# bytedance/ps-lite

Measured on AMD Instinct MI355X. Metric: push+pull GB/s per worker + p50 round-trip µs, 1 MB & 64 MB, at 1/2/4/8 GPUs, higher is better.
Workload: dtype fp32; 1 GPU; model=dense push+pull (ps-lite test_benchmark PUSH_PULL), global_batch=128, seq_len=67108864, parallelism=byteps-joint x1 (worker+server per GPU), mode=dense, msg_bytes=67108864, batch_keys=False, overlap=True, op=assign

## Files before the change

### csrc/gpu_plane.cc

```cpp
#include "gpu_plane.h"

#include <fcntl.h>
#include <hip/hip_runtime.h>
#include <semaphore.h>
#include <sys/prctl.h>
#include <time.h>
#include <unistd.h>

#include <cstring>

#include "hip_pool.h"
#include "host_par.h"
#include "host_pool.h"
#include "kernels.h"
#include "postoffice.h"
#include "wire.h"

namespace xps {

static const size_t kInlineMax = 4096;

#define XPS_HIP_CHECK(cmd)                                                            \
  do {                                                                                \
    hipError_t e_ = (cmd);                                                            \
    XPS_CHECK(e_ == hipSuccess) << "HIP error: " << hipGetErrorString(e_) << " in " #cmd; \
  } while (0)

std::atomic<uint64_t> g_zero_copy_recv{0};
std::atomic<uint64_t> g_fused_assign{0};

bool FusedAssignEnabled() {
  static const bool on = Environment::Get()->GetInt("XPS_FUSED_ASSIGN", 1) != 0;
  return on;
}

namespace {
std::mutex g_map_mu;
struct HandleKey {
  char h[kIpcHandleBytes];
  bool operator==(const HandleKey& o) const { return memcmp(h, o.h, kIpcHandleBytes) == 0; }
};
struct HandleHash {
  size_t operator()(const HandleKey& k) const {
    size_t v = 1469598103934665603ull;
    for (char c : k.h) {
      v ^= static_cast<unsigned char>(c);
      v *= 1099511628211ull;
    }
    return v;
  }
};
std::unordered_map<HandleKey, void*, HandleHash> g_mapped;

class IpcOpenLock {
 public:
  IpcOpenLock() {
    sem_ = sem_open("/xps_ipc_open_lock", O_CREAT, 0600, 1);
  }
  void Lock() {
// ... 4 lines not shown
    if (sem_timedwait(sem_, &ts) != 0) {
      XPS_LOG(Warning) << "ipc-open lock timeout; proceeding unlocked";
      timed_out_ = true;
    }
  }
  void Unlock() {
    if (sem_ != SEM_FAILED && !timed_out_) sem_post(sem_);
    timed_out_ = false;
  }

 private:
  sem_t* sem_ = SEM_FAILED;
  bool timed_out_ = false;
};
IpcOpenLock g_ipc_lock;
}

GpuPlane::GpuPlane(Postoffice* po, int device) : po_(po), device_(device) {
  my_host_hash_ = HostHash();
  inline_deliver_ = Environment::Get()->GetInt("XPS_INLINE_HANDLER", 1) != 0;
  lanes_ = Environment::Get()->GetInt("XPS_STREAMS_PER_PEER", 2);
  if (lanes_ < 1) lanes_ = 1;
  if (lanes_ > 2) lanes_ = 2;
}

GpuPlane::~GpuPlane() { Stop(); }

void GpuPlane::FillSelf(Node* self) {
  static std::once_flag gc_once;
  std::call_once(gc_once, [] { HostShmPool::GcStaleSegments(); });
  self->dev_id = device_;
  auto* pool = HbmPool::Get();
  if (device_ >= 0 && pool->initialized()) {
    self->pool_capacity = pool->capacity();
    self->pool_slab_bytes = pool->slab_bytes();
    self->pool_handles.resize(pool->slab_count());
    for (size_t i = 0; i < pool->slab_count(); ++i) {
      memcpy(self->pool_handles[i].data(), pool->slab_handle(i), kIpcHandleBytes);
    }
  }
  auto* hpool = HostShmPool::Get();
  hpool->Init(self->shm_uid);
  self->host_pool_uid = hpool->uid();
  self->host_pool_capacity = hpool->capacity();
  if (!started_) {
    auto* env = Environment::Get();
// ... 1 lines not shown
      XPS_CHECK(in_ring_.Create(self->shm_uid)) << "cannot create shm ring";
    }
    started_ = true;
    if (!env->GetInt("XPS_PROBE_NO_POLL", 0)) {
      poll_running_ = true;
      poll_thread_ = std::thread([this] { RingPollLoop(); });
    }
    if (device_ >= 0 && !env->GetInt("XPS_PROBE_NO_COMP", 0)) {
      comp_thread_ = std::thread([this] { CompletionLoop(); });
    }
  }
}

void GpuPlane::Stop() {
  if (stop_.exchange(true)) return;
  PrintStageStats(device_ >= 0 ? "gpu plane" : "host plane");
  if (poll_thread_.joinable()) poll_thread_.join();
  if (comp_thread_.joinable()) comp_thread_.join();
  {
    std::lock_guard<std::mutex> lk(local_mu_);
    for (auto& lm : local_q_) po_->van()->Deliver(std::move(lm.first));
    local_q_.clear();
  }
  {
    std::lock_guard<std::mutex> lk(pend_mu_);
    for (auto& kv : pending_) {
      for (auto& p : kv.second) {
        (void)hipEventSynchronize(p.ev);
        if (p.local_po) {
          DeliverLocal(p.local_po, p.resend, p.bytes);
          (void)hipEventDestroy(p.ev);
          continue;
        }
        Peer* peer = GetPeer(p.peer_id);
        auto ring = peer ? RingOf(peer) : nullptr;
        bool sent = ring && ring->Push(p.payload.data(),
                                       static_cast<uint32_t>(p.payload.size()));
        if (!sent) {
          (void)po_->van()->SendOverTcp(p.resend, p.peer_id);
        }
        (void)hipEventDestroy(p.ev);
      }
    }
    pending_.clear();
  }
  in_ring_.CloseAndUnlink();
  HostShmPool::Get()->Unlink();
  std::lock_guard<std::mutex> lk(ev_mu_);
  for (auto ev : event_pool_) (void)hipEventDestroy(ev);
  event_pool_.clear();
// ... 158 lines not shown
  std::lock_guard<std::mutex> lk(p->mu);
  p->slab_bases = std::move(bases);
  return !p->slab_bases.empty();
}

char* GpuPlane::ResolvePeer(Peer* p, uint64_t global_off, uint64_t len) {
  if (!ImportPeerSlabs(p)) return nullptr;
  uint64_t slab_bytes = p->node.pool_slab_bytes;
  if (slab_bytes == 0) return nullptr;
  size_t idx = static_cast<size_t>(global_off / slab_bytes);
  uint64_t local = global_off % slab_bytes;
  std::lock_guard<std::mutex> lk(p->mu);
  if (idx >= p->slab_bases.size() || len > slab_bytes - local) {
    XPS_LOG(Warning) << "peer offset out of bounds: off=" << global_off << " len=" << len
                     << " slab=" << idx;
    return nullptr;
  }
  return static_cast<char*>(p->slab_bases[idx]) + local;
}

hipStream_t GpuPlane::StreamLane(int node_id, int lane) {
  if (lane >= lanes_) lane = lanes_ - 1;
  Peer* p = GetPeer(node_id);
  hipStream_t s = p->streams[lane].load(std::memory_order_acquire);
  if (s) return s;
  std::lock_guard<std::mutex> lk(p->mu);
  s = p->streams[lane].load(std::memory_order_relaxed);
  if (!s) {
    XPS_HIP_CHECK(hipSetDevice(device_));
    XPS_HIP_CHECK(hipStreamCreateWithFlags(&s, hipStreamNonBlocking));
    p->streams[lane].store(s, std::memory_order_release);
  }
  return s;
}

hipStream_t GpuPlane::StreamForPeer(int node_id) { return StreamLane(node_id, 0); }

hipStream_t GpuPlane::PullStreamForPeer(int node_id) {
  Peer* p = GetPeer(node_id);
  if (lanes_ < 2 || p->node.dev_id == device_) return StreamLane(node_id, 0);
  return StreamLane(node_id, 1);
}

std::vector<std::tuple<int, int64_t, int64_t>> GpuPlane::PeerBytes() {
  std::vector<std::tuple<int, int64_t, int64_t>> out;
  std::shared_lock<std::shared_timed_mutex> lk(peers_mu_);
  for (auto& kv : peers_) {
    int64_t tx = kv.second->tx_bytes.load(std::memory_order_relaxed);
    int64_t rx = kv.second->rx_bytes.load(std::memory_order_relaxed);
    if (tx || rx) out.emplace_back(kv.first, tx, rx);
  }
  return out;
}

hipEvent_t GpuPlane::GetEvent() {
  {
    std::lock_guard<std::mutex> lk(ev_mu_);
    if (!event_pool_.empty()) {
      hipEvent_t ev = event_pool_.back();
      event_pool_.pop_back();
      return ev;
    }
  }
// ... 153 lines not shown
  }
  pending_count_.fetch_add(1);
  p->rx_bytes.fetch_add(bytes, std::memory_order_relaxed);
  return true;
}

bool GpuPlane::EntryPushPull(Message& msg, Peer* p, int64_t* bytes_out) {
  if (!FusedAssignEnabled()) return false;
  if (!(msg.meta.option & kOptPullAddr) || (msg.meta.option & kOptHostAddr)) return false;
  static const bool local_one_sided =
      Environment::Get()->GetInt("XPS_LOCAL_ONE_SIDED", 0) != 0;
  Postoffice* elpo = LocalPeer(p);
  GpuPlane* rplane =
      elpo ? dynamic_cast<GpuPlane*>(elpo->van() ? elpo->van()->plane() : nullptr) : nullptr;
  bool can = elpo ? (local_one_sided && rplane != nullptr) : EnsureRing(p);
  if (!can) return false;
  SArray<char> vals = msg.data[1];
  size_t len = vals.size();
  if (len == 0) return false;
  char* entry = ResolvePeer(p, msg.meta.entry_addr, len);
  char* dst = static_cast<char*>(HbmPool::Get()->PtrOf(msg.meta.addr, len));
  if (!entry || !dst || !kern::Disjoint3(entry, dst, vals.data(), len)) return false;
  XPS_STAGE(entry_push_pull);
  hipStream_t stream = elpo ? rplane->StreamForPeer(po_->node_id()) : StreamForPeer(p->node.id);
  XPS_HIP_CHECK(hipSetDevice(device_));
  kern::DenseAssign2(entry, dst, vals.data(), len, stream);
  g_fused_assign.fetch_add(1, std::memory_order_relaxed);
  g_zero_copy_recv.fetch_add(1, std::memory_order_relaxed);
  Message meta_msg;
  meta_msg.meta = msg.meta;
  meta_msg.meta.option |= kOptInPlace;
  meta_msg.meta.val_len = static_cast<int64_t>(len);
  meta_msg.meta.data_type.clear();
  for (size_t i = 0; i < msg.data.size(); ++i) {
    if (i == 1 || msg.data[i].on_device()) continue;
    meta_msg.data.push_back(msg.data[i]);
    meta_msg.meta.data_type.push_back(msg.meta.data_type[i]);
  }
  int64_t bytes = 64 + static_cast<int64_t>(len);
  Message keepalive;
  keepalive.data.push_back(vals);
  std::string payload;
  if (!elpo) {
    std::vector<char> br(meta_msg.data.size(), 0);
    XPS_CHECK(Serialize(meta_msg, br, &payload));
  }
  hipEvent_t ev = GetEvent();
  XPS_HIP_CHECK(hipEventRecord(ev, stream));
  {
    std::lock_guard<std::mutex> lk(pend_mu_);
    pending_[p->node.id].push_back(Pending{ev, p->node.id, std::move(payload),
                                           std::move(meta_msg), std::move(keepalive), bytes,
                                           elpo});
  }
  pending_count_.fetch_add(1);
  p->tx_bytes.fetch_add(bytes, std::memory_order_relaxed);
  *bytes_out = bytes;
  return true;
}

void GpuPlane::EnqueueLocal(Message msg, int64_t bytes) {
  {
    std::lock_guard<std::mutex> lk(local_mu_);
    local_q_.emplace_back(std::move(msg), bytes);
  }
  local_count_.fetch_add(1, std::memory_order_release);
}

int64_t GpuPlane::SendLocal(Message& msg, Peer* p, Postoffice* lpo) {
  XPS_STAGE(plane_send_local);
  bool response = !msg.meta.request;
  int64_t bytes = 64;
  for (auto& d : msg.data) bytes += static_cast<int64_t>(d.size());

  if (response && msg.meta.pull && msg.data.size() > 1 && !msg.data[1].on_device() &&
      msg.data[1].size() > 0 && (msg.meta.option & kOptPullAddr) &&
// ... 44 lines not shown
      if (i == 1 || msg.data[i].on_device()) continue;
      meta_msg.data.push_back(msg.data[i]);
      meta_msg.meta.data_type.push_back(msg.meta.data_type[i]);
    }
    msg.data.clear();
    Message keepalive;
    keepalive.data.push_back(vals);
    hipEvent_t ev = GetEvent();
    XPS_HIP_CHECK(hipEventRecord(ev, stream));
    {
      std::lock_guard<std::mutex> lk(pend_mu_);
      pending_[p->node.id].push_back(Pending{ev, p->node.id, std::string(),
                                             std::move(meta_msg), std::move(keepalive), bytes,
                                             lpo});
    }
    pending_count_.fetch_add(1);
    p->tx_bytes.fetch_add(bytes, std::memory_order_relaxed);
    return bytes;
  }

  bool kernel_less_ack = KernelLessAck(msg);
  if (response && device_ >= 0 && !kernel_less_ack) {
    XPS_STAGE(local_defer);
    hipStream_t stream = (msg.meta.option & kOptPullLane) ? PullStreamForPeer(p->node.id)
                                                          : StreamForPeer(p->node.id);
    hipEvent_t ev = GetEvent();
    XPS_HIP_CHECK(hipSetDevice(device_));
    XPS_HIP_CHECK(hipEventRecord(ev, stream));
    Message resend = msg;
    {
      std::lock_guard<std::mutex> lk(pend_mu_);
      pending_[p->node.id].push_back(Pending{ev, p->node.id, std::string(), std::move(resend),
                                             Message(), bytes, lpo});
    }
    pending_count_.fetch_add(1);
  } else {
    Message copy = msg;
    if (response) {
      for (auto& d : copy.data) {
        if (!d.on_device() && d.size()) {
          SArray<char> snap(d.size());
          memcpy(snap.data(), d.data(), d.size());
          d = snap;
        }
      }
    }
    DeliverLocal(lpo, copy, bytes);
  }
  p->tx_bytes.fetch_add(bytes, std::memory_order_relaxed);
  return bytes;
}

int64_t GpuPlane::Send(Message& msg, const Node& peer_node) {
  XPS_STAGE(plane_send);
  XPS_VLOG(3) << "plane send -> " << peer_node.id << ": " << msg.DebugString();
  Peer* p = GetPeer(peer_node.id);
// ... 195 lines not shown
  pending_count_.fetch_add(1);
  XPS_VLOG(3) << "deferred send queued -> " << peer_id;
}

void GpuPlane::CompletionLoop() {
  XPS_HIP_CHECK(hipSetDevice(device_));
  prctl(PR_SET_TIMERSLACK, 1000);
  const int kSpin = Environment::Get()->GetInt("XPS_POLL_SPIN", 200000);
  int idle = 0;
  std::vector<int> ids;
  while (!stop_.load()) {
    bool did = false;
    if (pending_count_.load(std::memory_order_acquire) > 0) {
      ids.clear();
      {
        std::lock_guard<std::mutex> lk(pend_mu_);
        for (auto& kv : pending_) {
          if (!kv.second.empty()) ids.push_back(kv.first);
        }
      }
      for (int id : ids) {
        while (!stop_.load()) {
          hipEvent_t front_ev = nullptr;
          {
            std::lock_guard<std::mutex> lk(pend_mu_);
            auto& dq = pending_[id];
            if (dq.empty()) break;
            front_ev = dq.front().ev;
          }
          hipError_t e = hipEventQuery(front_ev);
          if (e == hipErrorNotReady) break;
          XPS_STAGE(defer_release);
          XPS_CHECK(e == hipSuccess) << "hipEventQuery: " << hipGetErrorString(e);
          Pending front;
          {
            std::lock_guard<std::mutex> lk(pend_mu_);
            auto& dq = pending_[id];
            front = std::move(dq.front());
            dq.pop_front();
          }
          pending_count_.fetch_sub(1);
          if (front.local_po) {
            DeliverLocal(front.local_po, front.resend, front.bytes);
            PutEvent(front.ev);
            did = true;
            continue;
          }
          Peer* peer = GetPeer(front.peer_id);
          auto ring = peer ? RingOf(peer) : nullptr;
          bool sent = ring && ring->Push(front.payload.data(),
                                         static_cast<uint32_t>(front.payload.size()));
          if (sent) {
            XPS_VLOG(3) << "deferred send done -> " << front.peer_id;
          } else {
            XPS_LOG(Warning) << "deferred plane send failed -> " << front.peer_id
                             << "; falling back to TCP";
            if (po_->van()->SendOverTcp(front.resend, front.peer_id) < 0) {
              XPS_LOG(Warning) << "TCP fallback to " << front.peer_id
                               << " failed too (peer dead?)";
            }
          }
          PutEvent(front.ev);
          did = true;
        }
      }
    }
    if (did) {
      idle = 0;
    } else if (++idle > kSpin) {
      usleep(20);
    }
  }
}

void GpuPlane::RingPollLoop() {
  if (device_ >= 0) XPS_HIP_CHECK(hipSetDevice(device_));
  prctl(PR_SET_TIMERSLACK, 1000);
  const int kSpin = Environment::Get()->GetInt("XPS_POLL_SPIN", 200000);
  std::vector<char> buf(ShmRing::MaxPayload());
  int idle = 0;
  std::deque<std::pair<Message, int64_t>> local;
  while (!stop_.load()) {
    if (local_count_.load(std::memory_order_acquire) > 0) {
      {
        std::lock_guard<std::mutex> lk(local_mu_);
// ... 98 lines not shown
```

### csrc/gpu_plane.h

```cpp
#pragma once

#include <hip/hip_runtime.h>

#include <atomic>
#include <deque>
#include <memory>
#include <shared_mutex>
#include <thread>
#include <tuple>
#include <unordered_map>
#include <vector>

#include "shm_ring.h"
#include "van.h"

namespace xps {

extern std::atomic<uint64_t> g_zero_copy_recv;
extern std::atomic<uint64_t> g_fused_assign;
bool FusedAssignEnabled();

class Postoffice;

class GpuPlane : public DataPlane {
 public:
  GpuPlane(Postoffice* po, int device);
  ~GpuPlane() override;

  void FillSelf(Node* self) override;
  void ImportPeers() override;
  bool CanSend(const Message& msg, const Node& peer) override;
  int64_t Send(Message& msg, const Node& peer) override;
  void OnPeer(const Node& peer) override;
  void Stop() override;

  hipStream_t StreamForPeer(int node_id);
  hipStream_t PullStreamForPeer(int node_id);
  int lanes() const { return lanes_; }
  std::vector<std::tuple<int, int64_t, int64_t>> PeerBytes();
  int device() const { return device_; }

  bool LocalPullRead(int peer_id, void* dst, uint64_t entry_off, size_t len, Message resp);
  hipEvent_t GetEvent();
  void PutEvent(hipEvent_t ev);
  char* PeerDst(int peer_id, uint64_t global_off, uint64_t len) {
    return ResolvePeer(GetPeer(peer_id), global_off, len);
  }

 private:
  struct Peer {
    Node node;
    std::atomic<Postoffice*> local_po{nullptr};
    std::shared_ptr<ShmRing> ring;
    bool ring_tried = false;
    std::atomic<bool> ring_ok{false};
    std::vector<void*> slab_bases;
    bool pool_tried = false;
    std::atomic<hipStream_t> streams[2] = {{nullptr}, {nullptr}};
    std::atomic<int64_t> tx_bytes{0};
    std::atomic<int64_t> rx_bytes{0};
    std::mutex mu;
  };

  struct Pending {
    hipEvent_t ev;
    int peer_id;
    std::string payload;
    Message resend;
    Message keepalive;
    int64_t bytes;
    Postoffice* local_po = nullptr;
  };

  Peer* GetPeer(int id);
  Postoffice* LocalPeer(Peer* p);
  int64_t SendLocal(Message& msg, Peer* p, Postoffice* lpo);
  void DeliverLocal(Postoffice* lpo, Message& msg, int64_t bytes);
  void EnqueueLocal(Message msg, int64_t bytes);
  bool EnsureRing(Peer* p);
  std::shared_ptr<ShmRing> RingOf(Peer* p);
  bool ImportPeerSlabs(Peer* p);
  char* ResolvePeer(Peer* p, uint64_t global_off, uint64_t len);
  bool Serialize(const Message& msg, const std::vector<char>& by_ref, std::string* out);
  void RingPollLoop();
  void CompletionLoop();
  hipStream_t StreamLane(int node_id, int lane);
  bool EntryPushPull(Message& msg, Peer* p, int64_t* bytes_out);
  void DeferSendInternal(Peer* p, int peer_id, hipStream_t stream, Message resend,
                         Message keepalive, std::string payload, int64_t bytes);

  Postoffice* po_;
  int device_;
  int lanes_ = 2;
  uint64_t my_host_hash_;
  ShmRing in_ring_;
  bool started_ = false;
  bool inline_deliver_ = true;

  std::shared_timed_mutex peers_mu_;
  std::unordered_map<int, std::unique_ptr<Peer>> peers_;

  std::thread poll_thread_;
  std::thread comp_thread_;
  std::atomic<bool> stop_{false};

  std::mutex pend_mu_;
  std::unordered_map<int, std::deque<Pending>> pending_;
  std::atomic<int> pending_count_{0};

  std::mutex local_mu_;
  std::deque<std::pair<Message, int64_t>> local_q_;
  std::atomic<int> local_count_{0};
  bool poll_running_ = false;

  std::mutex ev_mu_;
  std::vector<hipEvent_t> event_pool_;
// ... 6 lines not shown
```

### csrc/kernels.h

```cpp
#pragma once

#include <cstddef>
#include <cstdint>

#include <hip/hip_runtime.h>

namespace xps {
namespace kern {

void DenseAssign(void* dst, const void* src, size_t nbytes, hipStream_t s);
void DenseAssign2(void* dst0, void* dst1, const void* src, size_t nbytes, hipStream_t s,
                  int grid_cap = 0);
inline bool Disjoint3(const void* a, const void* b, const void* c, size_t len) {
  auto apart = [len](const void* x, const void* y) {
    uintptr_t p = reinterpret_cast<uintptr_t>(x), q = reinterpret_cast<uintptr_t>(y);
    return p + len <= q || q + len <= p;
  };
  return apart(a, b) && apart(a, c) && apart(b, c);
}
void DenseSumF32(float* dst, const float* src, size_t n, hipStream_t s);
void DenseSumBf16(uint16_t* dst, const uint16_t* src, size_t n, hipStream_t s);
void BatchedSumBf16(const struct CopyDesc* descs_host, int n, hipStream_t s);
void SparseGatherF32(const float* table, const uint64_t* rows_dev, size_t nrows, size_t row_len,
                     float* out, hipStream_t s, int key_shift = 0, uint64_t row_base = 0,
                     uint64_t table_rows = ~0ull);
void SparseScatterAddF32(float* table, const uint64_t* rows_dev, size_t nrows, size_t row_len,
                         const float* src, bool atomic, hipStream_t s, int key_shift = 0,
                         uint64_t row_base = 0, uint64_t table_rows = ~0ull);
void SparseScatterAssignF32(float* table, const uint64_t* rows_dev, size_t nrows, size_t row_len,
                            const float* src, hipStream_t s, int key_shift = 0,
                            uint64_t row_base = 0, uint64_t table_rows = ~0ull);

static const int kMaxBatch = 64;
struct CopyDesc {
  void* dst;
  const void* src;
  size_t nbytes;
};
void BatchedAssign(const CopyDesc* descs_host, int n, hipStream_t s);
void BatchedSumF32(const CopyDesc* descs_host, int n, hipStream_t s);

}
}
```

### csrc/kernels.hip

```cpp
#include <hip/hip_runtime.h>

#include <algorithm>
#include <cstdlib>

#include "kernels.h"

namespace xps {
namespace kern {

namespace {

constexpr int kBlock = 256;

inline int GridFor(size_t work_items, int cap = 8192) {
  size_t g = (work_items + kBlock - 1) / kBlock;
  if (g > static_cast<size_t>(cap)) g = cap;
  if (g == 0) g = 1;
  return static_cast<int>(g);
}

__global__ void assign_kernel(uint4* __restrict__ dst, const uint4* __restrict__ src, size_t n4) {
  size_t i = blockIdx.x * static_cast<size_t>(blockDim.x) + threadIdx.x;
  size_t stride = static_cast<size_t>(gridDim.x) * blockDim.x;
  for (; i < n4; i += stride) dst[i] = src[i];
// ... 229 lines not shown
      float4 b = *src;
      a.x += b.x;
      a.y += b.y;
      a.z += b.z;
      a.w += b.w;
      *dst = a;
    } else if (kOp == 2) {
      uint4* dst = reinterpret_cast<uint4*>(da.d[seg].dst) + local;
      const uint4* src = reinterpret_cast<const uint4*>(da.d[seg].src) + local;
      uint4 a = *dst;
      uint4 b = *src;
      a.x = bf16x2_sum(a.x, b.x);
      a.y = bf16x2_sum(a.y, b.y);
      a.z = bf16x2_sum(a.z, b.z);
      a.w = bf16x2_sum(a.w, b.w);
      *dst = a;
    } else {
      reinterpret_cast<uint4*>(da.d[seg].dst)[local] =
          reinterpret_cast<const uint4*>(da.d[seg].src)[local];
    }
  }
}

__global__ void batched_assign_kernel(DescArray da) {
  for (int seg = 0; seg < da.n; ++seg) {
    uint4* dst = reinterpret_cast<uint4*>(da.d[seg].dst);
    const uint4* src = reinterpret_cast<const uint4*>(da.d[seg].src);
    size_t n4 = da.d[seg].nbytes / 16;
    size_t i = blockIdx.x * static_cast<size_t>(blockDim.x) + threadIdx.x;
    size_t stride = static_cast<size_t>(gridDim.x) * blockDim.x;
    for (; i < n4; i += stride) dst[i] = src[i];
  }
}

__global__ void batched_sum_kernel_bf16(DescArray da) {
  for (int seg = 0; seg < da.n; ++seg) {
    uint4* dst = reinterpret_cast<uint4*>(da.d[seg].dst);
    const uint4* src = reinterpret_cast<const uint4*>(da.d[seg].src);
    size_t n8 = da.d[seg].nbytes / 16;
    size_t i = blockIdx.x * static_cast<size_t>(blockDim.x) + threadIdx.x;
    size_t stride = static_cast<size_t>(gridDim.x) * blockDim.x;
    for (; i < n8; i += stride) {
      uint4 d = dst[i];
      uint4 s = src[i];
      d.x = bf16x2_sum(d.x, s.x);
      d.y = bf16x2_sum(d.y, s.y);
// ... 53 lines not shown
    int grid = static_cast<int>((acc + cpb - 1) / cpb);
    hipLaunchKernelGGL((batched_balanced_kernel<kOp>), dim3(grid), dim3(kBlock), 0, s, da,
                       cpb);
  }
}

}

void BatchedAssign(const CopyDesc* descs_host, int n, hipStream_t s) {
  if (BalancedBatchEnabled()) {
    LaunchBalanced<0>(descs_host, n, s);
    return;
  }
  size_t total = 0;
  for (int i = 0; i < n; ++i) total += descs_host[i].nbytes;
  DescArray da{};
  for (int off = 0; off < n; off += kMaxBatch) {
    da.n = std::min(n - off, kMaxBatch);
    for (int i = 0; i < da.n; ++i) da.d[i] = descs_host[off + i];
    hipLaunchKernelGGL(batched_assign_kernel, dim3(GridFor(total / 16)), dim3(kBlock), 0, s, da);
  }
}

void BatchedSumF32(const CopyDesc* descs_host, int n, hipStream_t s) {
  if (BalancedBatchEnabled()) {
    LaunchBalanced<1>(descs_host, n, s);
    return;
  }
  size_t total = 0;
  for (int i = 0; i < n; ++i) total += descs_host[i].nbytes;
  DescArray da{};
  for (int off = 0; off < n; off += kMaxBatch) {
    da.n = std::min(n - off, kMaxBatch);
    for (int i = 0; i < da.n; ++i) da.d[i] = descs_host[off + i];
    hipLaunchKernelGGL(batched_sum_kernel_f32, dim3(GridFor(total / 16)), dim3(kBlock), 0, s, da);
  }
}

void DenseAssign(void* dst, const void* src, size_t nbytes, hipStream_t s) {
  size_t n4 = nbytes / 16;
  if (n4) {
    hipLaunchKernelGGL(assign_kernel, dim3(GridFor(n4)), dim3(kBlock), 0, s,
                       static_cast<uint4*>(dst), static_cast<const uint4*>(src), n4);
  }
  if (nbytes % 16) {
    hipLaunchKernelGGL(assign_tail_kernel, dim3(1), dim3(kBlock), 0, s, static_cast<char*>(dst),
// ... 101 lines not shown
```

### csrc/pybind.cc

```cpp
#include <pybind11/functional.h>
#include <pybind11/numpy.h>
#include <pybind11/pybind11.h>
#include <pybind11/stl.h>

#include <atomic>
#include <thread>

#include "gpu_plane.h"
#include "hip_pool.h"
#include "hip_util.h"
#include "host_pool.h"
#include "kernels.h"
#include "kv_app.h"
#include "kv_utils.h"
#include "ps.h"
#include "server_handlers.h"
#include "shm_ring.h"
#include "simple_app.h"
#include "van.h"
#include "wire.h"

namespace py = pybind11;
using namespace xps;

// ... 499 lines not shown
      .def("round", &PyKVWorker::Round, py::arg("keys"), py::arg("ptrs"), py::arg("nbytes"),
           py::arg("device"), py::arg("cmd") = 0, py::arg("pull") = false)
      .def("round_mixed", &PyKVWorker::RoundMixed, py::arg("keys"), py::arg("push_ptrs"),
           py::arg("pull_ptrs"), py::arg("sizes"), py::arg("device"), py::arg("cmd") = 0,
           py::arg("overlap") = true);

  py::class_<PyKVServer>(m, "KVServer")
      .def(py::init<int, int>(), py::arg("app_id") = 0, py::arg("instance_idx") = 0)
      .def("set_default_handle", &PyKVServer::SetDefaultHandle)
      .def("set_reduce_handle", &PyKVServer::SetReduceHandle, py::arg("num_workers"))
      .def("set_gpu_dense_handle", &PyKVServer::SetGpuDenseHandle, py::arg("mode") = "assign",
           py::arg("dtype") = "f32")
      .def("set_gpu_sparse_handle", &PyKVServer::SetGpuSparseHandle, py::arg("rows"),
           py::arg("row_len"), py::arg("accumulate") = true, py::arg("key_shift") = 0)
      .def("register_entry", &PyKVServer::RegisterEntry, py::arg("key"), py::arg("ptr"),
           py::arg("nbytes"), py::arg("device") = 0)
      .def("sparse_table_ptr", &PyKVServer::SparseTablePtr)
      .def("save_checkpoint", &PyKVServer::SaveCheckpoint)
      .def("load_checkpoint", &PyKVServer::LoadCheckpoint)
      .def("set_python_handle", &PyKVServer::SetPythonHandle);

  m.def("zero_copy_recv_count", []() { return g_zero_copy_recv.load(); });
  m.def("fused_assign_count", []() { return g_fused_assign.load(); });

  m.def("plane_peer_bytes", [](const std::string& role, int idx) {
    py::dict out;
    auto* po = GetPO(role, idx);
    auto* plane = po->van() ? dynamic_cast<GpuPlane*>(po->van()->plane()) : nullptr;
    if (plane) {
      for (auto& t : plane->PeerBytes()) {
        out[py::int_(std::get<0>(t))] = py::make_tuple(std::get<1>(t), std::get<2>(t));
      }
    }
    return out;
  }, py::arg("role") = "worker", py::arg("idx") = 0);

  m.def("_order_nodes", [](std::vector<std::tuple<std::string, std::string, int>> in) {
    std::vector<Node> nodes;
    for (auto& t : in) {
      Node n;
      n.role = std::get<0>(t) == "worker" ? Node::WORKER : Node::SERVER;
      n.hostname = std::get<1>(t);
      n.port = std::get<2>(t);
      nodes.push_back(n);
    }
    auto less = NodeRankOrder(nodes);
// ... 193 lines not shown
        py::arg("src_keys"), py::arg("src_vals"), py::arg("dst_keys"), py::arg("k") = 1,
        py::arg("accumulate") = false, py::arg("nthreads") = 4);
  m.def("parallel_sort", [](py::array_t<uint64_t> keys, int nthreads) {
    SArray<Key> k;
    k.CopyFrom(keys.data(), keys.size());
    ParallelSort(&k, nthreads);
    py::array_t<uint64_t> out(k.size());
    std::copy(k.begin(), k.end(), out.mutable_data());
    return out;
  }, py::arg("keys"), py::arg("nthreads") = 4);

  m.def("k_dense_assign", [](uintptr_t dst, uintptr_t src, size_t nbytes) {
    kern::DenseAssign(reinterpret_cast<void*>(dst), reinterpret_cast<void*>(src), nbytes, nullptr);
    gpu::DeviceSync(-1);
  });
  m.def("k_dense_assign2",
        [](uintptr_t dst0, uintptr_t dst1, uintptr_t src, size_t nbytes, int grid_cap) {
          kern::DenseAssign2(reinterpret_cast<void*>(dst0), reinterpret_cast<void*>(dst1),
                             reinterpret_cast<void*>(src), nbytes, nullptr, grid_cap);
          gpu::DeviceSync(-1);
        },
        py::arg("dst0"), py::arg("dst1"), py::arg("src"), py::arg("nbytes"),
        py::arg("grid_cap") = 0);
  m.def("k_dense_sum_f32", [](uintptr_t dst, uintptr_t src, size_t n) {
    kern::DenseSumF32(reinterpret_cast<float*>(dst), reinterpret_cast<float*>(src), n, nullptr);
    gpu::DeviceSync(-1);
  });
  m.def("k_dense_sum_bf16", [](uintptr_t dst, uintptr_t src, size_t n) {
    kern::DenseSumBf16(reinterpret_cast<uint16_t*>(dst), reinterpret_cast<uint16_t*>(src), n,
                       nullptr);
    gpu::DeviceSync(-1);
  });
  m.def("k_sparse_gather_f32",
        [](uintptr_t table, uintptr_t rows, size_t nrows, size_t row_len, uintptr_t out) {
          kern::SparseGatherF32(reinterpret_cast<float*>(table),
                                reinterpret_cast<uint64_t*>(rows), nrows, row_len,
                                reinterpret_cast<float*>(out), nullptr);
          gpu::DeviceSync(-1);
        });
  m.def("k_sparse_scatter_add_f32",
        [](uintptr_t table, uintptr_t rows, size_t nrows, size_t row_len, uintptr_t src,
           bool atomic) {
          kern::SparseScatterAddF32(reinterpret_cast<float*>(table),
                                    reinterpret_cast<uint64_t*>(rows), nrows, row_len,
                                    reinterpret_cast<float*>(src), atomic, nullptr);
          gpu::DeviceSync(-1);
// ... 11 lines not shown
```

### csrc/server_handlers.cc

```cpp
#include "server_handlers.h"

#include "gpu_plane.h"
#include "hip_pool.h"
#include "kernels.h"

namespace xps {

#define XPS_HIP_CHECK(cmd)                                                            \
  do {                                                                                \
    hipError_t e_ = (cmd);                                                            \
    XPS_CHECK(e_ == hipSuccess) << "HIP error: " << hipGetErrorString(e_) << " in " #cmd; \
  } while (0)

static GpuPlane* ThePlane(Postoffice* po) {
  return dynamic_cast<GpuPlane*>(po->van() ? po->van()->plane() : nullptr);
}

static hipStream_t PeerStream(Postoffice* po, int sender, hipStream_t* fallback) {
  auto* plane = ThePlane(po);
  if (plane) return plane->StreamForPeer(sender);
  if (!*fallback) {
    XPS_HIP_CHECK(hipStreamCreateWithFlags(fallback, hipStreamNonBlocking));
  }
  return *fallback;
// ... 37 lines not shown
  chain_ = num_workers_ > 1;
}

void GpuDenseHandler::SumKernel(void* dst, const void* src, size_t nbytes, hipStream_t s) {
  if (dtype_ == DenseDtype::kBf16) {
    kern::DenseSumBf16(static_cast<uint16_t*>(dst), static_cast<const uint16_t*>(src),
                       nbytes / 2, s);
  } else {
    kern::DenseSumF32(static_cast<float*>(dst), static_cast<const float*>(src), nbytes / 4, s);
  }
}

void GpuDenseHandler::BatchedSum(const kern::CopyDesc* descs, int n, hipStream_t s) {
  if (dtype_ == DenseDtype::kBf16) {
    kern::BatchedSumBf16(descs, n, s);
  } else {
    kern::BatchedSumF32(descs, n, s);
  }
}

bool GpuDenseHandler::NeedChain(int sender) {
  if (chain_) return true;
  auto* plane = ThePlane(po_);
  return plane && plane->lanes() > 1 &&
         plane->PullStreamForPeer(sender) != plane->StreamForPeer(sender);
}

GpuDenseHandler::~GpuDenseHandler() = default;

void GpuDenseHandler::OrderAfter(Entry* e, hipStream_t s) {
  if (e->last_ev) XPS_HIP_CHECK(hipStreamWaitEvent(s, e->last_ev.get(), 0));
}

hipStream_t GpuDenseHandler::Stream(int sender) {
  return PeerStream(po_, sender, &fallback_stream_);
}

hipStream_t GpuDenseHandler::PullStream(int sender) {
  return PeerPullStream(po_, sender, &fallback_stream_);
}

void GpuDenseHandler::operator()(const KVMeta& req, const KVPairs<float>& kvs,
                                 KVServer<float>* server) {
  if (req.push && req.pull) {
    XPS_CHECK(mode_ != DenseMode::kReduce)
        << "ZPushPull is not supported in reduce mode (pulls are held per round)";
    if (req.option & kOptInPlace) {
      server->Response(req);
// ... 23 lines not shown
                                : static_cast<size_t>(kvs.lens[0]) * sizeof(float);
  if (len == 0 || len != kvs.vals.nbytes() || static_cast<int64_t>(len) != req.val_len) {
    return false;
  }
  auto* plane = ThePlane(po_);
  if (!plane) return false;
  char* dst = plane->PeerDst(req.sender, req.addr, len);
  if (!dst) return false;
  XPS_STAGE(dense_fused_assign);
  XPS_HIP_CHECK(hipSetDevice(HbmPool::Get()->device()));
  Entry* e;
  {
    std::lock_guard<std::mutex> lk(mu_);
    e = &store_[kvs.keys[0]];
    if (e->buf.size() < len) {
      if (!e->buf.empty()) e->retired.push_back(e->buf);
      e->buf = HbmPool::Get()->AllocArray(len);
      XPS_HIP_CHECK(hipMemset(e->buf.data(), 0, len));
    }
  }
  if (e->buf.size() != len) return false;
  const char* src = reinterpret_cast<const char*>(kvs.vals.data());
  if (!kern::Disjoint3(e->buf.data(), dst, src, len)) return false;
  hipStream_t stream = Stream(req.sender);
  OrderAfter(e, stream);
  kern::DenseAssign2(e->buf.data(), dst, src, len, stream);
  g_fused_assign.fetch_add(1, std::memory_order_relaxed);
  g_zero_copy_recv.fetch_add(1, std::memory_order_relaxed);
  if (NeedChain(req.sender)) e->last_ev = MakeEventRef(po_, stream);
  KVMeta r = req;
  r.option |= kOptInPlace;
  r.option &= ~(kOptPullLane | kOptEntryPush);
  r.val_len = static_cast<int64_t>(len);
  uint64_t eoff = 0;
  if (HbmPool::Get()->OffsetOf(e->buf.data(), &eoff)) {
    r.entry_addr = eoff;
    r.option |= kOptEntryAddr;
  }
  server->Response(r);
  return true;
}

GpuDenseHandler::Group* GpuDenseHandler::GroupFor(const SArray<Key>& keys) {
  uint64_t h = 1469598103934665603ull;
  const unsigned char* p = reinterpret_cast<const unsigned char*>(keys.data());
  for (size_t i = 0; i < keys.nbytes(); ++i) {
    h ^= p[i];
    h *= 1099511628211ull;
  }
  Group* g;
  {
    std::lock_guard<std::mutex> lk(mu_);
    g = &groups_[h];
  }
  if (g->keys.empty()) {
    g->keys.assign(keys.begin(), keys.end());
    g->ents.reserve(keys.size());
    std::lock_guard<std::mutex> lk(mu_);
    for (Key k : g->keys) g->ents.push_back(&store_[k]);
  } else {
    XPS_CHECK(g->keys.size() == keys.size() &&
              std::equal(g->keys.begin(), g->keys.end(), keys.begin()))
// ... 583 lines not shown
```

Baseline: 3465 GB/s.

## Coalesce per-peer fused assign launches into batched kernel with shared completion events

```diff
diff --git a/csrc/coalesce_admit.h b/csrc/coalesce_admit.h
--- /dev/null
+++ b/csrc/coalesce_admit.h
@@ -0,0 +1,57 @@
+#pragma once
+
+#include <cstddef>
+#include <cstdint>
+
+namespace xps {
+namespace kern {
+
+struct Seg2 {
+  void* dst0;
+  void* dst1;
+  const void* src;
+  size_t nbytes;
+};
+
+static const int kMaxBatch2 = 64;
+
+enum class Admit {
+  kAdmit,
+  kFlushFirst,
+  kReject,
+};
+
+inline bool RangesOverlap(const void* a, const void* b, size_t alen, size_t blen) {
+  uintptr_t p = reinterpret_cast<uintptr_t>(a), q = reinterpret_cast<uintptr_t>(b);
+  return p < q + blen && q < p + alen;
+}
+
+inline Admit CoalesceAdmit(const Seg2* open, int n_open, const Seg2& s) {
+  uintptr_t bits = reinterpret_cast<uintptr_t>(s.dst0) | reinterpret_cast<uintptr_t>(s.dst1) |
+                   reinterpret_cast<uintptr_t>(s.src) | static_cast<uintptr_t>(s.nbytes);
+  if (s.nbytes == 0 || (bits & 15u) != 0) return Admit::kReject;
+  if (RangesOverlap(s.dst0, s.dst1, s.nbytes, s.nbytes) ||
+      RangesOverlap(s.dst0, s.src, s.nbytes, s.nbytes) ||
+      RangesOverlap(s.dst1, s.src, s.nbytes, s.nbytes)) {
+    return Admit::kReject;
+  }
+  if (n_open >= kMaxBatch2) return Admit::kReject;
+  for (int i = 0; i < n_open; ++i) {
+    const Seg2& o = open[i];
+    const void* theirs[3] = {o.dst0, o.dst1, o.src};
+    for (const void* t : theirs) {
+      if (RangesOverlap(s.dst0, t, s.nbytes, o.nbytes) ||
+          RangesOverlap(s.dst1, t, s.nbytes, o.nbytes)) {
+        return Admit::kFlushFirst;
+      }
+    }
+    if (RangesOverlap(s.src, o.dst0, s.nbytes, o.nbytes) ||
+        RangesOverlap(s.src, o.dst1, s.nbytes, o.nbytes)) {
+      return Admit::kFlushFirst;
+    }
+  }
+  return Admit::kAdmit;
+}
+
+}
+}
diff --git a/csrc/gpu_plane.cc b/csrc/gpu_plane.cc
--- a/csrc/gpu_plane.cc
+++ b/csrc/gpu_plane.cc
@@ -34,7 +34,29 @@
   return on;
 }
 
+std::atomic<uint64_t> g_fused_launches{0};
+
+bool CoalesceEnabled() {
+  static const bool on = Environment::Get()->GetInt("XPS_COALESCE", 1) != 0;
+  return on;
+}
+
 namespace {
+struct CoTicket {
+  const void* plane = nullptr;
+  int peer = 0;
+  std::shared_ptr<void> cev;
+};
+thread_local CoTicket t_co_ticket;
+
+int64_t NowUs() {
+  struct timespec ts;
+  clock_gettime(CLOCK_MONOTONIC, &ts);
+  return static_cast<int64_t>(ts.tv_sec) * 1000000 + ts.tv_nsec / 1000;
+}
+const int64_t kHoldQuietUs = 2000;
+const size_t kCoBusyBytes = 16u << 20;
+
 std::mutex g_map_mu;
 struct HandleKey {
   char h[kIpcHandleBytes];
@@ -85,6 +107,9 @@
   lanes_ = Environment::Get()->GetInt("XPS_STREAMS_PER_PEER", 2);
   if (lanes_ < 1) lanes_ = 1;
   if (lanes_ > 2) lanes_ = 2;
+  co_hold_ = Environment::Get()->GetInt("XPS_COALESCE_HOLD", 0) != 0;
+  int cap_mb = Environment::Get()->GetInt("XPS_COALESCE_CAP_MB", 1024);
+  co_byte_cap_ = static_cast<size_t>(cap_mb < 1 ? 1 : cap_mb) << 20;
 }
 
 GpuPlane::~GpuPlane() { Stop(); }
@@ -132,10 +157,36 @@
     for (auto& lm : local_q_) po_->van()->Deliver(std::move(lm.first));
     local_q_.clear();
   }
+  if (device_ >= 0) {
+    std::vector<Peer*> all;
+    {
+      std::shared_lock<std::shared_timed_mutex> lk(peers_mu_);
+      for (auto& kv : peers_) all.push_back(kv.second.get());
+    }
+    for (Peer* peer : all) {
+      CoFlush(peer);
+      std::lock_guard<std::mutex> lk(peer->co.mu);
+      peer->co.inflight.clear();
+    }
+  }
   {
     std::lock_guard<std::mutex> lk(pend_mu_);
     for (auto& kv : pending_) {
       for (auto& p : kv.second) {
+        if (p.cev) {
+          (void)hipEventSynchronize(p.cev->ev.load(std::memory_order_acquire));
+          if (p.local_po) {
+            DeliverLocal(p.local_po, p.resend, p.bytes);
+          } else {
+            Peer* peer = GetPeer(p.peer_id);
+            auto ring = peer ? RingOf(peer) : nullptr;
+            if (!ring || !ring->Push(p.payload.data(),
+                                     static_cast<uint32_t>(p.payload.size()))) {
+              (void)po_->van()->SendOverTcp(p.resend, p.peer_id);
+            }
+          }
+          continue;
+        }
         (void)hipEventSynchronize(p.ev);
         if (p.local_po) {
           DeliverLocal(p.local_po, p.resend, p.bytes);
@@ -340,6 +391,127 @@
 hipStream_t GpuPlane::StreamLane(int node_id, int lane) {
   if (lane >= lanes_) lane = lanes_ - 1;
   Peer* p = GetPeer(node_id);
+  if (lane == 0) CoFlush(p);
+  return RawLane(p, lane);
+}
+
+bool GpuPlane::LanesSplit(int node_id) {
+  return lanes_ >= 2 && GetPeer(node_id)->node.dev_id != device_;
+}
+
+
+void GpuPlane::CoLaunchLocked(Peer* p) {
+  Coalescer& co = p->co;
+  if (co.n == 0) return;
+  hipStream_t stream = RawLane(p, 0);
+  XPS_HIP_CHECK(hipSetDevice(device_));
+  if (co.n == 1) {
+    const kern::Seg2& s = co.segs[0];
+    kern::DenseAssign2(s.dst0, s.dst1, s.src, s.nbytes, stream);
+  } else {
+    kern::BatchedAssign2(co.segs, co.n, stream);
+  }
+  g_fused_launches.fetch_add(1, std::memory_order_relaxed);
+  hipEvent_t ev = GetEvent();
+  XPS_HIP_CHECK(hipEventRecord(ev, stream));
+  co.open->bytes = co.bytes;
+  co.open->ev.store(ev, std::memory_order_release);
+  co.inflight.push_back(std::move(co.open));
+  co.open.reset();
+  co.n = 0;
+  co.bytes = 0;
+  co.n_open.store(0, std::memory_order_release);
+}
+
+bool GpuPlane::CoBusyLocked(Peer* p) {
+  CoPruneLocked(p);
+  size_t bytes = 0;
+  for (auto& f : p->co.inflight) bytes += f->bytes;
+  return p->co.inflight.size() >= 2 && bytes >= kCoBusyBytes;
+}
+
+void GpuPlane::CoPruneLocked(Peer* p) {
+  auto& fl = p->co.inflight;
+  while (!fl.empty()) {
+    CoEvent* f = fl.front().get();
+    if (!f->done.load(std::memory_order_acquire) &&
+        hipEventQuery(f->ev.load(std::memory_order_acquire)) != hipSuccess) {
+      break;
+    }
+    fl.pop_front();
+  }
+}
+
+void GpuPlane::CoFlush(Peer* p) {
+  if (p->co.n_open.load(std::memory_order_acquire) == 0) return;
+  std::lock_guard<std::mutex> lk(p->co.mu);
+  CoLaunchLocked(p);
+}
+
+std::shared_ptr<GpuPlane::CoEvent> GpuPlane::CoAppend(Peer* p, const kern::Seg2& seg) {
+  if (!CoalesceEnabled()) return nullptr;
+  Coalescer& co = p->co;
+  std::lock_guard<std::mutex> lk(co.mu);
+  kern::Admit a = kern::CoalesceAdmit(co.segs, co.n, seg);
+  if (a != kern::Admit::kAdmit) CoLaunchLocked(p);
+  if (a == kern::Admit::kReject) return nullptr;
+  if (!co.open) co.open = std::make_shared<CoEvent>(this);
+  std::shared_ptr<CoEvent> cev = co.open;
+  co.segs[co.n++] = seg;
+  co.bytes += seg.nbytes;
+  co.n_open.store(co.n, std::memory_order_release);
+  if (co.n >= kern::kMaxBatch || co.bytes >= co_byte_cap_) {
+    CoLaunchLocked(p);
+  } else if (co_hold_) {
+    co.last_append_us = NowUs();
+  } else {
+    if (!CoBusyLocked(p)) CoLaunchLocked(p);
+  }
+  return cev;
+}
+
+bool GpuPlane::CoFrontUnlaunched(Peer* p, const std::shared_ptr<CoEvent>& cev) {
+  Coalescer& co = p->co;
+  std::lock_guard<std::mutex> lk(co.mu);
+  if (co.open != cev) return true;
+  if (co_hold_ && NowUs() - co.last_append_us < kHoldQuietUs) return false;
+  CoLaunchLocked(p);
+  return true;
+}
+
+void GpuPlane::CoRetired(Peer* p) {
+  Coalescer& co = p->co;
+  std::lock_guard<std::mutex> lk(co.mu);
+  bool busy = CoBusyLocked(p);
+  if (!co_hold_ && !busy) CoLaunchLocked(p);
+}
+
+bool GpuPlane::CoalesceAppend(int peer_id, const kern::Seg2& seg) {
+  if (device_ < 0) return false;
+  std::shared_ptr<CoEvent> cev = CoAppend(GetPeer(peer_id), seg);
+  if (!cev) return false;
+  t_co_ticket.plane = this;
+  t_co_ticket.peer = peer_id;
+  t_co_ticket.cev = std::move(cev);
+  return true;
+}
+
+std::shared_ptr<GpuPlane::CoEvent> GpuPlane::TakeTicket(int peer_id) {
+  if (!t_co_ticket.cev || t_co_ticket.plane != this || t_co_ticket.peer != peer_id) {
+    return nullptr;
+  }
+  auto cev = std::static_pointer_cast<CoEvent>(t_co_ticket.cev);
+  t_co_ticket.cev.reset();
+  return cev;
+}
+
+void GpuPlane::CoalesceEnd(int peer_id) {
+  if (!t_co_ticket.cev) return;
+  t_co_ticket.cev.reset();
+  CoFlush(GetPeer(peer_id));
+}
+
+hipStream_t GpuPlane::RawLane(Peer* p, int lane) {
   hipStream_t s = p->streams[lane].load(std::memory_order_acquire);
   if (s) return s;
   std::lock_guard<std::mutex> lk(p->mu);
@@ -357,6 +529,7 @@
 hipStream_t GpuPlane::PullStreamForPeer(int node_id) {
   Peer* p = GetPeer(node_id);
   if (lanes_ < 2 || p->node.dev_id == device_) return StreamLane(node_id, 0);
+  CoFlush(p);
   return StreamLane(node_id, 1);
 }
 
@@ -556,9 +729,17 @@
   char* dst = static_cast<char*>(HbmPool::Get()->PtrOf(msg.meta.addr, len));
   if (!entry || !dst || !kern::Disjoint3(entry, dst, vals.data(), len)) return false;
   XPS_STAGE(entry_push_pull);
-  hipStream_t stream = elpo ? rplane->StreamForPeer(po_->node_id()) : StreamForPeer(p->node.id);
-  XPS_HIP_CHECK(hipSetDevice(device_));
-  kern::DenseAssign2(entry, dst, vals.data(), len, stream);
+  std::shared_ptr<CoEvent> cev;
+  static const bool co_one_sided =
+      Environment::Get()->GetInt("XPS_COALESCE_ONE_SIDED", 0) != 0;
+  if (!elpo && co_one_sided) cev = CoAppend(p, kern::Seg2{entry, dst, vals.data(), len});
+  hipStream_t stream = nullptr;
+  if (!cev) {
+    stream = elpo ? rplane->StreamForPeer(po_->node_id()) : StreamForPeer(p->node.id);
+    XPS_HIP_CHECK(hipSetDevice(device_));
+    kern::DenseAssign2(entry, dst, vals.data(), len, stream);
+    g_fused_launches.fetch_add(1, std::memory_order_relaxed);
+  }
   g_fused_assign.fetch_add(1, std::memory_order_relaxed);
   g_zero_copy_recv.fetch_add(1, std::memory_order_relaxed);
   Message meta_msg;
@@ -579,13 +760,16 @@
     std::vector<char> br(meta_msg.data.size(), 0);
     XPS_CHECK(Serialize(meta_msg, br, &payload));
   }
-  hipEvent_t ev = GetEvent();
-  XPS_HIP_CHECK(hipEventRecord(ev, stream));
+  hipEvent_t ev = nullptr;
+  if (!cev) {
+    ev = GetEvent();
+    XPS_HIP_CHECK(hipEventRecord(ev, stream));
+  }
   {
     std::lock_guard<std::mutex> lk(pend_mu_);
     pending_[p->node.id].push_back(Pending{ev, p->node.id, std::move(payload),
                                            std::move(meta_msg), std::move(keepalive), bytes,
-                                           elpo});
+                                           elpo, std::move(cev)});
   }
   pending_count_.fetch_add(1);
   p->tx_bytes.fetch_add(bytes, std::memory_order_relaxed);
@@ -676,16 +860,20 @@
   bool kernel_less_ack = KernelLessAck(msg);
   if (response && device_ >= 0 && !kernel_less_ack) {
     XPS_STAGE(local_defer);
-    hipStream_t stream = (msg.meta.option & kOptPullLane) ? PullStreamForPeer(p->node.id)
-                                                          : StreamForPeer(p->node.id);
-    hipEvent_t ev = GetEvent();
-    XPS_HIP_CHECK(hipSetDevice(device_));
-    XPS_HIP_CHECK(hipEventRecord(ev, stream));
+    std::shared_ptr<CoEvent> cev = TakeTicket(p->node.id);
+    hipEvent_t ev = nullptr;
+    if (!cev) {
+      hipStream_t stream = (msg.meta.option & kOptPullLane) ? PullStreamForPeer(p->node.id)
+                                                            : StreamForPeer(p->node.id);
+      ev = GetEvent();
+      XPS_HIP_CHECK(hipSetDevice(device_));
+      XPS_HIP_CHECK(hipEventRecord(ev, stream));
+    }
     Message resend = msg;
     {
       std::lock_guard<std::mutex> lk(pend_mu_);
       pending_[p->node.id].push_back(Pending{ev, p->node.id, std::string(), std::move(resend),
-                                             Message(), bytes, lpo});
+                                             Message(), bytes, lpo, std::move(cev)});
     }
     pending_count_.fetch_add(1);
   } else {
@@ -927,16 +1115,33 @@
       for (int id : ids) {
         while (!stop_.load()) {
           hipEvent_t front_ev = nullptr;
+          std::shared_ptr<CoEvent> cev;
           {
             std::lock_guard<std::mutex> lk(pend_mu_);
             auto& dq = pending_[id];
             if (dq.empty()) break;
             front_ev = dq.front().ev;
+            cev = dq.front().cev;
           }
-          hipError_t e = hipEventQuery(front_ev);
-          if (e == hipErrorNotReady) break;
+          bool retired = false;
+          if (cev) {
+            front_ev = cev->ev.load(std::memory_order_acquire);
+            if (!front_ev) {
+              if (!CoFrontUnlaunched(GetPeer(id), cev)) break;
+              continue;
+            }
+          }
+          if (!cev || !cev->done.load(std::memory_order_acquire)) {
+            hipError_t e = hipEventQuery(front_ev);
+            if (e == hipErrorNotReady) break;
+            XPS_CHECK(e == hipSuccess) << "hipEventQuery: " << hipGetErrorString(e);
+            if (cev) {
+              cev->done.store(true, std::memory_order_release);
+              retired = true;
+            }
+          }
           XPS_STAGE(defer_release);
-          XPS_CHECK(e == hipSuccess) << "hipEventQuery: " << hipGetErrorString(e);
+          if (retired) CoRetired(GetPeer(id));
           Pending front;
           {
             std::lock_guard<std::mutex> lk(pend_mu_);
@@ -947,7 +1152,7 @@
           pending_count_.fetch_sub(1);
           if (front.local_po) {
             DeliverLocal(front.local_po, front.resend, front.bytes);
-            PutEvent(front.ev);
+            if (front.ev) PutEvent(front.ev);
             did = true;
             continue;
           }
@@ -965,7 +1170,7 @@
                                << " failed too (peer dead?)";
             }
           }
-          PutEvent(front.ev);
+          if (front.ev) PutEvent(front.ev);
           did = true;
         }
       }
diff --git a/csrc/gpu_plane.h b/csrc/gpu_plane.h
--- a/csrc/gpu_plane.h
+++ b/csrc/gpu_plane.h
@@ -11,6 +11,7 @@
 #include <unordered_map>
 #include <vector>
 
+#include "kernels.h"
 #include "shm_ring.h"
 #include "van.h"
 
@@ -19,6 +20,8 @@
 extern std::atomic<uint64_t> g_zero_copy_recv;
 extern std::atomic<uint64_t> g_fused_assign;
 bool FusedAssignEnabled();
+extern std::atomic<uint64_t> g_fused_launches;
+bool CoalesceEnabled();
 
 class Postoffice;
 
@@ -37,6 +40,10 @@
   hipStream_t StreamForPeer(int node_id);
   hipStream_t PullStreamForPeer(int node_id);
   int lanes() const { return lanes_; }
+  bool LanesSplit(int node_id);
+
+  bool CoalesceAppend(int peer_id, const kern::Seg2& seg);
+  void CoalesceEnd(int peer_id);
   std::vector<std::tuple<int, int64_t, int64_t>> PeerBytes();
   int device() const { return device_; }
 
@@ -48,8 +55,30 @@
   }
 
  private:
+  struct CoEvent {
+    explicit CoEvent(GpuPlane* pl) : plane(pl) {}
+    ~CoEvent() {
+      if (hipEvent_t e = ev.load(std::memory_order_acquire)) plane->PutEvent(e);
+    }
+    GpuPlane* plane;
+    std::atomic<hipEvent_t> ev{nullptr};
+    std::atomic<bool> done{false};
+    size_t bytes = 0;
+  };
+  struct Coalescer {
+    std::mutex mu;
+    kern::Seg2 segs[kern::kMaxBatch];
+    int n = 0;
+    std::atomic<int> n_open{0};
+    size_t bytes = 0;
+    std::shared_ptr<CoEvent> open;
+    std::deque<std::shared_ptr<CoEvent>> inflight;
+    int64_t last_append_us = 0;
+  };
+
   struct Peer {
     Node node;
+    Coalescer co;
     std::atomic<Postoffice*> local_po{nullptr};
     std::shared_ptr<ShmRing> ring;
     bool ring_tried = false;
@@ -70,6 +99,7 @@
     Message keepalive;
     int64_t bytes;
     Postoffice* local_po = nullptr;
+    std::shared_ptr<CoEvent> cev;
   };
 
   Peer* GetPeer(int id);
@@ -85,6 +115,15 @@
   void RingPollLoop();
   void CompletionLoop();
   hipStream_t StreamLane(int node_id, int lane);
+  hipStream_t RawLane(Peer* p, int lane);
+  std::shared_ptr<CoEvent> CoAppend(Peer* p, const kern::Seg2& seg);
+  void CoLaunchLocked(Peer* p);
+  void CoPruneLocked(Peer* p);
+  bool CoBusyLocked(Peer* p);
+  void CoFlush(Peer* p);
+  bool CoFrontUnlaunched(Peer* p, const std::shared_ptr<CoEvent>& cev);
+  void CoRetired(Peer* p);
+  std::shared_ptr<CoEvent> TakeTicket(int peer_id);
   bool EntryPushPull(Message& msg, Peer* p, int64_t* bytes_out);
   void DeferSendInternal(Peer* p, int peer_id, hipStream_t stream, Message resend,
                          Message keepalive, std::string payload, int64_t bytes);
@@ -92,6 +131,8 @@
   Postoffice* po_;
   int device_;
   int lanes_ = 2;
+  bool co_hold_ = false;
+  size_t co_byte_cap_ = 1ull << 30;
   uint64_t my_host_hash_;
   ShmRing in_ring_;
   bool started_ = false;
diff --git a/csrc/kernels.h b/csrc/kernels.h
--- a/csrc/kernels.h
+++ b/csrc/kernels.h
@@ -4,6 +4,8 @@
 #include <cstdint>
 
 #include <hip/hip_runtime.h>
+
+#include "coalesce_admit.h"
 
 namespace xps {
 namespace kern {
@@ -40,5 +42,8 @@
 void BatchedAssign(const CopyDesc* descs_host, int n, hipStream_t s);
 void BatchedSumF32(const CopyDesc* descs_host, int n, hipStream_t s);
 
+static_assert(kMaxBatch2 == kMaxBatch, "Seg2 batches use the batched kernels' segment limit");
+void BatchedAssign2(const Seg2* segs_host, int n, hipStream_t s, int tile_cap = 0);
+
 }
 }
diff --git a/csrc/kernels.hip b/csrc/kernels.hip
--- a/csrc/kernels.hip
+++ b/csrc/kernels.hip
@@ -275,6 +275,55 @@
   }
 }
 
+struct Seg2Array {
+  Seg2 d[kMaxBatch];
+  unsigned long long prefix[kMaxBatch + 1];
+  int n;
+};
+
+__global__ void batched_assign2_kernel(Seg2Array da, size_t chunks_per_block) {
+  size_t total = da.prefix[da.n];
+  size_t first = blockIdx.x * chunks_per_block;
+  size_t end = first + chunks_per_block;
+  if (end > total) end = total;
+  if (first >= end) return;
+  const size_t step = blockDim.x;
+  size_t begin = first + threadIdx.x;
+  int seg = 0;
+  {
+    int lo = 0, hi = da.n - 1;
+    while (lo < hi) {
+      int mid = (lo + hi + 1) >> 1;
+      if (da.prefix[mid] <= first) {
+        lo = mid;
+      } else {
+        hi = mid - 1;
+      }
+    }
+    seg = lo;
+  }
+  size_t seg_lo = da.prefix[seg], seg_hi = da.prefix[seg + 1];
+  uint4* d0 = static_cast<uint4*>(da.d[seg].dst0);
+  uint4* d1 = static_cast<uint4*>(da.d[seg].dst1);
+  const uint4* sp = static_cast<const uint4*>(da.d[seg].src);
+  for (size_t g = begin; g < end; g += step) {
+    if (g >= seg_hi) {
+      do {
+        ++seg;
+        seg_hi = da.prefix[seg + 1];
+      } while (g >= seg_hi);
+      seg_lo = da.prefix[seg];
+      d0 = static_cast<uint4*>(da.d[seg].dst0);
+      d1 = static_cast<uint4*>(da.d[seg].dst1);
+      sp = static_cast<const uint4*>(da.d[seg].src);
+    }
+    size_t local = g - seg_lo;
+    uint4 v = sp[local];
+    d0[local] = v;
+    d1[local] = v;
+  }
+}
+
 __global__ void batched_assign_kernel(DescArray da) {
   for (int seg = 0; seg < da.n; ++seg) {
     uint4* dst = reinterpret_cast<uint4*>(da.d[seg].dst);
@@ -374,6 +423,29 @@
   }
 }
 
+void BatchedAssign2(const Seg2* segs_host, int n, hipStream_t s, int tile_cap) {
+  int max_blocks = tile_cap > 0 ? std::min(tile_cap, 8192) : 8192;
+  int off = 0;
+  while (off < n) {
+    Seg2Array da{};
+    unsigned long long acc = 0;
+    while (off < n && da.n < kMaxBatch) {
+      const Seg2& sg = segs_host[off++];
+      if (sg.nbytes < 16) continue;
+      da.d[da.n] = sg;
+      da.prefix[da.n] = acc;
+      acc += sg.nbytes / 16;
+      ++da.n;
+    }
+    da.prefix[da.n] = acc;
+    if (acc == 0) continue;
+    size_t cpb = (acc + max_blocks - 1) / max_blocks;
+    cpb = ((cpb + kBlock - 1) / kBlock) * kBlock;
+    int grid = static_cast<int>((acc + cpb - 1) / cpb);
+    hipLaunchKernelGGL(batched_assign2_kernel, dim3(grid), dim3(kBlock), 0, s, da, cpb);
+  }
+}
+
 void BatchedSumF32(const CopyDesc* descs_host, int n, hipStream_t s) {
   if (BalancedBatchEnabled()) {
     LaunchBalanced<1>(descs_host, n, s);
diff --git a/csrc/pybind.cc b/csrc/pybind.cc
--- a/csrc/pybind.cc
+++ b/csrc/pybind.cc
@@ -545,6 +545,24 @@
 
   m.def("zero_copy_recv_count", []() { return g_zero_copy_recv.load(); });
   m.def("fused_assign_count", []() { return g_fused_assign.load(); });
+  m.def("fused_assign_launches", []() { return g_fused_launches.load(); });
+  m.def("coalesce_admit",
+        [](const std::vector<std::tuple<uintptr_t, uintptr_t, uintptr_t, size_t>>& open,
+           const std::tuple<uintptr_t, uintptr_t, uintptr_t, size_t>& seg) {
+          auto conv = [](const std::tuple<uintptr_t, uintptr_t, uintptr_t, size_t>& t) {
+            return kern::Seg2{reinterpret_cast<void*>(std::get<0>(t)),
+                              reinterpret_cast<void*>(std::get<1>(t)),
+                              reinterpret_cast<const void*>(std::get<2>(t)), std::get<3>(t)};
+          };
+          std::vector<kern::Seg2> segs;
+          for (auto& t : open) segs.push_back(conv(t));
+          switch (kern::CoalesceAdmit(segs.data(), static_cast<int>(segs.size()), conv(seg))) {
+            case kern::Admit::kAdmit: return "admit";
+            case kern::Admit::kFlushFirst: return "flush";
+            default: return "reject";
+          }
+        },
+        py::arg("open"), py::arg("seg"));
 
   m.def("plane_peer_bytes", [](const std::string& role, int idx) {
     py::dict out;
@@ -784,6 +802,26 @@
         },
         py::arg("dst0"), py::arg("dst1"), py::arg("src"), py::arg("nbytes"),
         py::arg("grid_cap") = 0);
+  m.def("k_batched_assign2",
+        [](const std::vector<std::tuple<uintptr_t, uintptr_t, uintptr_t, size_t>>& segs,
+           int tile_cap) {
+          std::vector<kern::Seg2> v;
+          for (auto& t : segs) {
+            v.push_back(kern::Seg2{reinterpret_cast<void*>(std::get<0>(t)),
+                                   reinterpret_cast<void*>(std::get<1>(t)),
+                                   reinterpret_cast<const void*>(std::get<2>(t)),
+                                   std::get<3>(t)});
+            if (kern::CoalesceAdmit(nullptr, 0, v.back()) != kern::Admit::kAdmit) {
+              throw std::invalid_argument("k_batched_assign2: segment " +
+                                          std::to_string(v.size() - 1) +
+                                          " is misaligned, not a 16 B multiple or "
+                                          "self-overlapping");
+            }
+          }
+          kern::BatchedAssign2(v.data(), static_cast<int>(v.size()), nullptr, tile_cap);
+          gpu::DeviceSync(-1);
+        },
+        py::arg("segs"), py::arg("tile_cap") = 0);
   m.def("k_dense_sum_f32", [](uintptr_t dst, uintptr_t src, size_t n) {
     kern::DenseSumF32(reinterpret_cast<float*>(dst), reinterpret_cast<float*>(src), n, nullptr);
     gpu::DeviceSync(-1);
diff --git a/csrc/server_handlers.cc b/csrc/server_handlers.cc
--- a/csrc/server_handlers.cc
+++ b/csrc/server_handlers.cc
@@ -83,8 +83,7 @@
 bool GpuDenseHandler::NeedChain(int sender) {
   if (chain_) return true;
   auto* plane = ThePlane(po_);
-  return plane && plane->lanes() > 1 &&
-         plane->PullStreamForPeer(sender) != plane->StreamForPeer(sender);
+  return plane && plane->LanesSplit(sender);
 }
 
 GpuDenseHandler::~GpuDenseHandler() = default;
@@ -154,12 +153,18 @@
   if (e->buf.size() != len) return false;
   const char* src = reinterpret_cast<const char*>(kvs.vals.data());
   if (!kern::Disjoint3(e->buf.data(), dst, src, len)) return false;
-  hipStream_t stream = Stream(req.sender);
-  OrderAfter(e, stream);
-  kern::DenseAssign2(e->buf.data(), dst, src, len, stream);
+  bool chain = NeedChain(req.sender);
+  bool coalesced = !chain && !e->last_ev &&
+                   plane->CoalesceAppend(req.sender, kern::Seg2{e->buf.data(), dst, src, len});
+  if (!coalesced) {
+    hipStream_t stream = Stream(req.sender);
+    OrderAfter(e, stream);
+    kern::DenseAssign2(e->buf.data(), dst, src, len, stream);
+    g_fused_launches.fetch_add(1, std::memory_order_relaxed);
+    if (chain) e->last_ev = MakeEventRef(po_, stream);
+  }
   g_fused_assign.fetch_add(1, std::memory_order_relaxed);
   g_zero_copy_recv.fetch_add(1, std::memory_order_relaxed);
-  if (NeedChain(req.sender)) e->last_ev = MakeEventRef(po_, stream);
   KVMeta r = req;
   r.option |= kOptInPlace;
   r.option &= ~(kOptPullLane | kOptEntryPush);
@@ -170,6 +175,7 @@
     r.option |= kOptEntryAddr;
   }
   server->Response(r);
+  if (coalesced) plane->CoalesceEnd(req.sender);
   return true;
 }
 
```

After: 3855 GB/s, median of 6. 1.11x the previous value.
